# MaurizioFD/RecSys2019_DeepLearning_Evaluation

Measured on NVIDIA H100. Metric: ItemKNN cosine top-K rows/sec, higher is better.
Workload: dtype i32 counts + f32

## Files before the change

### recsys2019_deeplearning_evaluation_b200/csrc/sim_k1d.cuh

```cuda

constexpr int D_THREADS = 512;
constexpr int D_WARPS = D_THREADS / 32;
constexpr int D_ROWS = 4;
constexpr int D_TILE_LOG2 = 10;

constexpr int K1D_GAPS = 6;
__device__ __forceinline__ int k1d_gap(const int4& c, int e) {
  const int w = e < 2 ? c.y : (e < 4 ? c.z : c.w);
  return (e & 1) ? (int)((unsigned)w >> 16) : (w & 0xffff);
}

struct K1DShared {
  int item, nbuf, cnt, nibsum, tstop, chunk_end, chunk_cnt;
  int ncand, expect;
  CtaSelectSmem<256> sel;
};

__device__ __forceinline__ unsigned nib_ge3(unsigned w) { return (((w | (w >> 1)) >> 2) | (w & (w >> 1))) & 0x11111111u; }
__device__ __forceinline__ unsigned nib_eq2(unsigned w) { return (w >> 1) & ~w & ~(w >> 2) & ~(w >> 3) & 0x11111111u; }
__device__ __forceinline__ unsigned nib_eq1(unsigned w) { return w & ~(w >> 1) & ~(w >> 2) & ~(w >> 3) & 0x11111111u; }
__device__ __forceinline__ unsigned nib_level(unsigned w, int level) {
  return level >= 3 ? nib_ge3(w) : (level == 2 ? nib_eq2(w) : nib_eq1(w));
}
__device__ __forceinline__ int nib_sum(unsigned w) {
  const unsigned b = (w & 0x0F0F0F0Fu) + ((w >> 4) & 0x0F0F0F0Fu);
  return (int)__dp4a(b, 0x01010101u, 0u);
}

__device__ u64 d_select(u64* buf, int n, int K, K1DShared* ds, int* n_out) {
  const int tid = threadIdx.x;
  __syncthreads();
  if (n <= K) { *n_out = n; return 0ull; }
  const auto sel_key = [&](int q, u64& key) {
    key = buf[q];
    return true;
  };
  const u64 thr = radix_select<u64, 8, true>(CtaSelect<D_THREADS, 256>(ds->sel), n, K, sel_key).thr;
  u64 keep[8];
#pragma unroll
  for (int q = 0; q < 8; ++q) {
    const int i = q * D_THREADS + tid;
    const u64 k = i < n ? buf[i] : 0ull;
    keep[q] = k >= thr ? k : 0ull;
  }
  if (tid == 0) ds->cnt = 0;
  __syncthreads();
#pragma unroll
  for (int q = 0; q < 8; ++q)
    if (keep[q]) buf[atomicAdd(&ds->cnt, 1)] = keep[q];
  __syncthreads();
  *n_out = ds->cnt;
  return thr;
}

template <int F>
__global__ void __launch_bounds__(D_THREADS, 2) sim_k1d_kernel(const KParams p) {
  extern __shared__ __align__(16) unsigned char smem_raw[];
  __shared__ K1DShared ds;
  const int tid = threadIdx.x, lane = tid & 31, warp = tid >> 5;
  const int W = p.bm_words;
  const int Wr = (p.n_cols + 7) >> 3;
  const int ntile = p.ntile;
  unsigned* acc = reinterpret_cast<unsigned*>(smem_raw);
  u64* buf = reinterpret_cast<u64*>(smem_raw + (size_t)W * 4);
  float* tbs = reinterpret_cast<float*>(buf + p.cap_d);
  int* tcnt = reinterpret_cast<int*>(tbs + ntile + 1);

  for (int i = tid; i < W; i += D_THREADS) acc[i] = 0u;
  for (int i = tid; i <= ntile; i += D_THREADS) tbs[i] = p.tbnd[i];
  for (int i = tid; i < ntile; i += D_THREADS) tcnt[i] = 0;
  long long prof_t = p.prof ? clock64() : 0;
  const int K = p.K;
  const int n_items = p.n_range_dev ? *p.n_range_dev : p.n_range;

  for (;;) {
    __syncthreads();
    if (tid == 0) { ds.item = atomicAdd(p.counter, 1); ds.nbuf = 0; ds.nibsum = 0; ds.ncand = 0; }
    __syncthreads();
    const int item = ds.item;
    if (item >= n_items) break;
    const int4 wi = __ldg(p.worklist + item);
    const int col = wi.x, lc = wi.y, cs = wi.z, ce = wi.w;
    const size_t out_base = (size_t)lc * K;
    const float Ai = p.A[col];
    const int adds = __ldg(p.col_adds + col);

    for (int k0 = cs + warp * 32; k0 < ce; k0 += D_WARPS * 32) {
      const int nrows = min(32, ce - k0);
      int2 seg = make_int2(0, 0);
      if (lane < nrows) seg = __ldg(p.csc_seg + k0 + lane);
      const int hl = lane & 15, hh = lane >> 4;
      for (int r0 = 0; r0 < nrows; r0 += 2 * D_ROWS) {
        int4 v[D_ROWS];
        int rs[D_ROWS], rn[D_ROWS];
#pragma unroll
        for (int q = 0; q < D_ROWS; ++q) {
          const int r = r0 + 2 * q + hh;
          rs[q] = __shfl_sync(0xffffffffu, seg.x, r & 31);
          rn[q] = __shfl_sync(0xffffffffu, seg.y, r & 31);
          if (r >= nrows) rn[q] = 0;
          if (hl < rn[q]) v[q] = __ldg(p.csr_idx1 + (size_t)rs[q] + hl);
        }
#pragma unroll
        for (int q = 0; q < D_ROWS; ++q) {
          int c0 = 0;
          for (;;) {
            if (c0 + hl < rn[q]) {
              int j = v[q].x;
              if (j < p.n_cols && j != col) atomicAdd(&acc[j >> 3], 1u << ((j & 7) << 2));
#pragma unroll
              for (int e = 0; e < K1D_GAPS; ++e) {
                const int g = k1d_gap(v[q], e);
                j += g;
                if (g && j < p.n_cols && j != col) atomicAdd(&acc[j >> 3], 1u << ((j & 7) << 2));
              }
            }
            c0 += 16;
            if (c0 >= rn[q]) break;
            if (c0 + hl < rn[q]) v[q] = __ldg(p.csr_idx1 + (size_t)rs[q] + c0 + hl);
          }
        }
      }
    }
    __syncthreads();
    PROF_MARK(1);

    {
      int ns = 0;
      unsigned* cand = reinterpret_cast<unsigned*>(buf);
      const int cand_cap = p.cap_d;
      const uint4* acc4 = reinterpret_cast<const uint4*>(acc);
      for (int i4 = tid; i4 < ((Wr + 3) >> 2); i4 += D_THREADS) {
        const uint4 w4 = acc4[i4];
        if (!(w4.x | w4.y | w4.z | w4.w)) continue;
        const unsigned ww[4] = {w4.x, w4.y, w4.z, w4.w};
        unsigned bytes = 0u, any = 0u, m[4];
#pragma unroll
        for (int e = 0; e < 4; ++e) {
          bytes += (ww[e] & 0x0F0F0F0Fu) + ((ww[e] >> 4) & 0x0F0F0F0Fu);
          m[e] = nib_ge3(ww[e]);
          any |= m[e];
        }
        ns += (int)__dp4a(bytes, 0x01010101u, 0u);
        if (any) {
          const int c3 = __popc(m[0]) + __popc(m[1]) + __popc(m[2]) + __popc(m[3]);
          atomicAdd(&tcnt[(i4 * 4) >> (D_TILE_LOG2 - 3)], c3);
          int pos = atomicAdd(&ds.ncand, c3);
          if (pos + c3 <= cand_cap) {
#pragma unroll
            for (int e = 0; e < 4; ++e) {
              unsigned mm = m[e];
              while (mm) {
                const int q = (__ffs(mm) - 1) >> 2;
                mm &= mm - 1;
                cand[pos++] = ((unsigned)((i4 * 4 + e) * 8 + q) << 4) | ((ww[e] >> (q << 2)) & 15u);
              }
            }
          }
        }
      }
      ns = __reduce_add_sync(0xffffffffu, ns);
      if (lane == 0 && ns) atomicAdd(&ds.nibsum, ns);
    }
    __syncthreads();
    const bool forced = p.fail_every > 0 && (lc % p.fail_every) == 0;
    if (ds.nibsum != adds || forced) {
      __syncthreads();
      if (tid == 0) p.redo[atomicAdd(p.fail, 1)] = lc;
      for (int i = tid; i < (W >> 2); i += D_THREADS) reinterpret_cast<int4*>(acc)[i] = make_int4(0, 0, 0, 0);
      for (int i = tid; i < ntile; i += D_THREADS) tcnt[i] = 0;
      continue;
    }
    PROF_MARK(2);

    u64 thr = 0ull;
    int n_have = 0;
    const int n3 = ds.ncand;
    const bool collected = n3 <= p.cap_d;
    if (collected) {
      const unsigned* cand = reinterpret_cast<const unsigned*>(buf);
      u64 keys[4];
#pragma unroll
      for (int q = 0; q < 4; ++q) {
        const int t = q * D_THREADS + tid;
        keys[q] = 0ull;
        if (t < n3) {
          const unsigned cd = cand[t];
          const int2 bn = __ldg(p.BN + (cd >> 4));
          const float sv = sim_value<F>(p, (float)(cd & 15u), Ai, __int_as_float(bn.x));
          if (sv > 0.f) keys[q] = (((u64)__float_as_uint(sv)) << 32) | (u64)(0xFFFFFFFFu - (unsigned)bn.y);
        }
      }
      __syncthreads();
#pragma unroll
      for (int q = 0; q < 4; ++q)
        if (keys[q]) buf[atomicAdd(&ds.nbuf, 1)] = keys[q];
      for (int i = tid; i < ntile; i += D_THREADS) tcnt[i] = 0;
      __syncthreads();
      n_have = ds.nbuf;
      if (n_have >= K) {
        const float fl = sim_value<F>(p, 3.f, Ai, tbs[ntile]) * (1.f - 1e-6f);
        if (fl > 0.f) thr = ((u64)__float_as_uint(fl)) << 32;
      }
      PROF_MARK(3);
    }
#pragma unroll 1
    for (int level = collected ? 2 : 3; level >= 1; --level) {
      int t_end = ntile;
      if (level < 3) {
        if (thr == 0ull) {
          t_end = ntile;
        } else {
          const float tsim = __uint_as_float((unsigned)(thr >> 32));
          if (tid == 0) ds.tstop = ntile;
          __syncthreads();
          for (int t = tid; t < ntile; t += D_THREADS)
            if (!(sim_value<F>(p, (float)level, Ai, tbs[t]) >= tsim)) atomicMin(&ds.tstop, t);
          __syncthreads();
          t_end = ds.tstop;
          __syncthreads();
        }
        if (t_end == 0) continue;
        const int w_end = min(Wr, t_end << (D_TILE_LOG2 - 3));
        for (int i = tid; i < w_end; i += D_THREADS) {
          const unsigned w = acc[i];
          if (!w) continue;
          const int c = __popc(nib_level(w, level));
          if (c) atomicAdd(&tcnt[i >> (D_TILE_LOG2 - 3)], c);
        }
        __syncthreads();
      }
      int t0 = 0;
      while (t0 < t_end) {
        if (tid == 0) {
          int t1 = t0, c = 0;
          while (t1 < t_end && n_have + c + tcnt[t1] <= p.cap_d) { c += tcnt[t1]; ++t1; }
          ds.chunk_end = t1;
          ds.chunk_cnt = c;
        }
        __syncthreads();
        const int t1 = ds.chunk_end;
        if (t1 == t0) {
          int kept;
          const u64 t2 = d_select(buf, n_have, K, &ds, &kept);
          thr = max(thr, t2);
          if (tid == 0) ds.nbuf = kept;
          n_have = kept;
          __syncthreads();
          continue;
        }
        if (ds.chunk_cnt > 0) {
          const int w_lo = t0 << (D_TILE_LOG2 - 3), w_hi = min(Wr, t1 << (D_TILE_LOG2 - 3));
          for (int i = w_lo + tid; i < w_hi; i += D_THREADS) {
            const unsigned w = acc[i];
            if (!w) continue;
            unsigned m = nib_level(w, level);
            while (m) {
              const int q = (__ffs(m) - 1) >> 2;
              m &= m - 1;
              const int j = i * 8 + q;
              const float d = (float)((w >> (q << 2)) & 15u);
              const int2 bn = __ldg(p.BN + j);
              const float sv = sim_value<F>(p, d, Ai, __int_as_float(bn.x));
              const u64 key = (((u64)__float_as_uint(sv)) << 32) | (u64)(0xFFFFFFFFu - (unsigned)bn.y);
              if (sv > 0.f && key >= thr) buf[atomicAdd(&ds.nbuf, 1)] = key;
            }
          }
        }
        __syncthreads();
        n_have = ds.nbuf;
        t0 = t1;
      }
      for (int i = tid; i < ntile; i += D_THREADS) tcnt[i] = 0;
      __syncthreads();
      if (n_have >= K) {
        if (level == 3 && thr == 0ull) {
          const float fl = sim_value<F>(p, 3.f, Ai, tbs[ntile]) * (1.f - 1e-6f);
          if (fl > 0.f) thr = ((u64)__float_as_uint(fl)) << 32;
        } else if (level == 2 && n_have > K) {
          int kept;
          const u64 t2 = d_select(buf, n_have, K, &ds, &kept);
          thr = max(thr, t2);
          if (tid == 0) ds.nbuf = kept;
          n_have = kept;
          __syncthreads();
        }
      }
      if (level == 3) PROF_MARK(3); else if (level == 2) PROF_MARK(4); else PROF_MARK(5);
    }

    {
      int kept;
      d_select(buf, n_have, K, &ds, &kept);
      n_have = kept;
    }
    for (int t = tid; t < n_have; t += D_THREADS) {
      const u64 k64 = buf[t];
      emit_entry(p, out_base + t, (int)(0xFFFFFFFFu - (unsigned)k64), __uint_as_float((unsigned)(k64 >> 32)));
    }
    for (int t = n_have + tid; t < K; t += D_THREADS) {
      emit_entry(p, out_base + t, -1, 0.f);
    }
    if (tid == 0) emit_count(p, lc, n_have);
    for (int i = tid; i < (W >> 2); i += D_THREADS) reinterpret_cast<int4*>(acc)[i] = make_int4(0, 0, 0, 0);
    PROF_MARK(6);
  }
}


#ifndef B200_U_THREADS
#define B200_U_THREADS 256
#endif
#ifndef B200_U_CTAS
#define B200_U_CTAS 4
#endif
#ifndef B200_U_STEPS
#define B200_U_STEPS 4
#endif
#ifndef B200_U_STAGE
#define B200_U_STAGE 1024
#endif
constexpr int U_THREADS = B200_U_THREADS;
constexpr int U_WARPS = U_THREADS / 32;
constexpr int U_CTAS = B200_U_CTAS;
constexpr int U_STEPS = B200_U_STEPS;
constexpr int U_STAGE = B200_U_STAGE;

__host__ __device__ __forceinline__ int k1d_window_size(int n, int c) { return ((n - 1) >> 1) + ((n & 1) == 0 && c < (n >> 1) ? 1 : 0); }
__host__ __device__ __forceinline__ int k1d_upper_words(int n) { return (((n >> 1) + 7) / 8 + 3) / 4 * 4; }
constexpr int OWN_SPILLED = (int)0x80000000u;

struct K1DUpShared {
  int item, nibsum, ncand, nst;
  unsigned long long base;
};

__global__ void __launch_bounds__(U_THREADS, U_CTAS) sim_k1d_upper_kernel(const KParams p) {
  extern __shared__ __align__(16) unsigned char smem_raw[];
  __shared__ K1DUpShared us;
  const int tid = threadIdx.x, lane = tid & 31, warp = tid >> 5;
  const int n = p.n_cols;
  const int W = k1d_upper_words(n);
  unsigned* acc = reinterpret_cast<unsigned*>(smem_raw);
  unsigned* stage = acc + W;
  for (int i = tid; i < W; i += U_THREADS) acc[i] = 0u;
  if (blockIdx.x == 0 && tid == 0 && p.fail_every > 0) atomicExch(p.pair_fail, 1);
  long long prof_t = p.prof ? clock64() : 0;

  for (;;) {
    __syncthreads();
    if (tid == 0) {
      us.item = *(volatile int*)p.pair_fail ? p.n_range : atomicAdd(p.counter, 1);
      us.nibsum = 0; us.ncand = 0; us.nst = 0;
    }
    __syncthreads();
    const int item = us.item;
    if (item >= p.n_range) break;
    const int4 wi = __ldg(p.worklist_up + item);
    const int col = wi.x, adds = wi.y, cs = wi.z, ce = wi.w;
    const int size_c = k1d_window_size(n, col);

    for (int k0 = cs + warp * 32; k0 < ce; k0 += U_WARPS * 32) {
      const int nrows = min(32, ce - k0);
      int2 seg = make_int2(0, 0);
      if (lane < nrows) seg = __ldg(p.csc_win + k0 + lane);
      const unsigned nz = __ballot_sync(0xffffffffu, seg.y > 0);
      const int nr = __popc(nz);
      const int src = lane < nr ? (int)__fns(nz, 0, lane + 1) : 0;
      const int rstart = __shfl_sync(0xffffffffu, seg.x, src);
      const int sy = __shfl_sync(0xffffffffu, seg.y, src);
      const int rn = lane < nr ? sy : 0;
      int end = rn;
#pragma unroll
      for (int off = 1; off < 32; off <<= 1) {
        const int t = __shfl_up_sync(0xffffffffu, end, off);
        if (lane >= off) end += t;
      }
      const int beg = end - rn;
      const int total = __shfl_sync(0xffffffffu, end, 31);
      for (int b0 = 0; b0 < total; b0 += 32 * U_STEPS) {
        int4 v[U_STEPS];
#pragma unroll
        for (int q = 0; q < U_STEPS; ++q) {
          const int base = b0 + 32 * q, f = base + lane;
          const unsigned before = __ballot_sync(0xffffffffu, lane < nr && end <= base);
          const unsigned ends = __reduce_or_sync(0xffffffffu, (lane < nr && end > base && end - base < 32) ? (1u << (end - base)) : 0u);
          const int row = (__popc(before) + __popc(ends & ((2u << lane) - 1u))) & 31;
          const int rb = __shfl_sync(0xffffffffu, beg, row), rs = __shfl_sync(0xffffffffu, rstart, row);
          if (f < total) v[q] = __ldg(p.csr_idx1 + (size_t)rs + (f - rb));
        }
#pragma unroll
        for (int q = 0; q < U_STEPS; ++q) {
          if (b0 + 32 * q + lane < total) {
            unsigned t = (unsigned)(v[q].x - col - 1);
            if (t < (unsigned)size_c) atomicAdd(&acc[t >> 3], 1u << ((t & 7) << 2));
#pragma unroll
            for (int e = 0; e < K1D_GAPS; ++e) {
              const unsigned g = (unsigned)k1d_gap(v[q], e);
              t += g;
              if (g && t < (unsigned)size_c) atomicAdd(&acc[t >> 3], 1u << ((t & 7) << 2));
            }
          }
        }
      }
    }
    __syncthreads();
    PROF_MARK(8);

    {
      int ns = 0;
      uint4* acc4 = reinterpret_cast<uint4*>(acc);
      for (int i4 = tid; i4 < ((((size_c + 7) >> 3) + 3) >> 2); i4 += U_THREADS) {
        const uint4 w4 = acc4[i4];
        if (!(w4.x | w4.y | w4.z | w4.w)) continue;
        acc4[i4] = make_uint4(0u, 0u, 0u, 0u);
        const unsigned ww[4] = {w4.x, w4.y, w4.z, w4.w};
        unsigned bytes = 0u, any = 0u, m[4];
#pragma unroll
        for (int e = 0; e < 4; ++e) {
          bytes += (ww[e] & 0x0F0F0F0Fu) + ((ww[e] >> 4) & 0x0F0F0F0Fu);
          m[e] = nib_ge3(ww[e]);
          any |= m[e];
        }
        ns += (int)__dp4a(bytes, 0x01010101u, 0u);
        if (any) {
          const int c3 = __popc(m[0]) + __popc(m[1]) + __popc(m[2]) + __popc(m[3]);
          int pos = atomicAdd(&us.ncand, c3);
          const bool staged = pos + c3 <= U_STAGE;
          unsigned long long g = 0ull;
          if (staged) atomicAdd(&us.nst, c3);
          else g = atomicAdd(p.n_loose, (unsigned long long)c3);
#pragma unroll
          for (int e = 0; e < 4; ++e) {
            unsigned mm = m[e];
            while (mm) {
              const int q = (__ffs(mm) - 1) >> 2;
              mm &= mm - 1;
              int j = col + 1 + (i4 * 4 + e) * 8 + q;
              if (j >= n) j -= n;
              const unsigned cd = ((unsigned)j << 4) | ((ww[e] >> (q << 2)) & 15u);
              if (staged) {
                stage[pos++] = cd;
              } else {
                atomicAdd(p.deg + j, 1);
                if (g < (unsigned long long)p.loose_cap) p.loose[g] = ((u64)col << 32) | cd;
                else atomicExch(p.pair_fail, 1);
                ++g;
              }
            }
          }
        }
      }
      ns = __reduce_add_sync(0xffffffffu, ns);
      if (lane == 0 && ns) atomicAdd(&us.nibsum, ns);
    }
    __syncthreads();
    const int nst = us.nst;
    if (tid == 0) {
      if (us.nibsum != adds) atomicExch(p.pair_fail, 1);
      us.base = nst ? atomicAdd(p.n_own, (unsigned long long)nst) : 0ull;
      if (us.base + nst > (unsigned long long)p.pair_cap) atomicExch(p.pair_fail, 1);
      p.own_off[col] = (int)us.base;
      p.own_n[col] = nst | (us.ncand > nst ? OWN_SPILLED : 0);
    }
    __syncthreads();
    const unsigned long long base = us.base;
    if (base + nst <= (unsigned long long)p.pair_cap)
      for (int t = tid; t < nst; t += U_THREADS) {
        const unsigned cd = stage[t];
        p.own[base + t] = cd;
        atomicAdd(p.deg + (cd >> 4), 1);
      }
    PROF_MARK(9);
  }
}

__global__ void k1d_pair_scatter_kernel(const KParams p) {
  const long long t0 = blockIdx.x * (long long)blockDim.x + threadIdx.x, nt = (long long)gridDim.x * blockDim.x;
  if (*p.pair_fail) {
    for (long long q = t0; q <= p.n_cols; q += nt) p.deg[q] = 0;
    return;
  }
  const int i = (int)(t0 >> 5), lane = threadIdx.x & 31;
  if (i < p.n_cols) {
    const int s = p.own_off[i], n = p.own_n[i] & ~OWN_SPILLED;
    for (int t = lane; t < n; t += 32) {
      const unsigned cd = p.own[s + t], j = cd >> 4;
      p.mir[p.mir_off[j] + atomicSub(p.deg + j, 1) - 1] = ((unsigned)i << 4) | (cd & 15u);
    }
  }
  const long long nl = (long long)min(*p.n_loose, (u64)p.loose_cap);
  for (long long q = t0; q < nl; q += nt) {
    const u64 e = p.loose[q];
    const unsigned cd = (unsigned)e, j = cd >> 4;
    p.mir[p.mir_off[j] + atomicSub(p.deg + j, 1) - 1] = ((unsigned)(e >> 32) << 4) | (cd & 15u);
  }
}

constexpr int S_WARPS = 4;
constexpr int S_CTAS = 6;
constexpr int S_CAP = 4 * D_THREADS;
constexpr int S_ILP = 12;
__host__ __device__ __forceinline__ int k1d_select_warp_bytes(int sel_cap) { return 256 * 4 + (sel_cap * 8 + 15) / 16 * 16; }

template <int F>
__global__ void __launch_bounds__(32 * S_WARPS, S_CTAS) sim_k1d_select_kernel(const KParams p) {
  extern __shared__ __align__(16) unsigned char smem_raw[];
  unsigned char* mine = smem_raw + (size_t)(threadIdx.x >> 5) * k1d_select_warp_bytes(p.sel_cap);
  int* hist = reinterpret_cast<int*>(mine);
  u64* keys = reinterpret_cast<u64*>(mine + 256 * 4);
  const int lane = threadIdx.x & 31;
  const int item = blockIdx.x * S_WARPS + (threadIdx.x >> 5);
  if (item >= p.n_range) return;
  const int4 wi = __ldg(p.worklist + item);
  if (*(volatile int*)p.pair_fail) {
    if (lane == 0) { p.wl_redo[item] = wi; atomicAdd(p.n_redo, 1); }
    return;
  }
  long long prof_t = p.prof ? clock64() : 0;
  const int col = wi.x, lc = wi.y, K = p.K;
  const int so = p.own_off[col], no = p.own_n[col];
  const int sm = p.mir_off[col], n = no + (p.mir_off[col + 1] - sm);
  bool ok = no >= 0 && n <= p.sel_cap;
  int n_have = 0;
  if (ok) {
    const float Ai = p.A[col];
    const unsigned* own = p.own + so;
    const unsigned* mir = p.mir + sm - no;
    for (int t0 = 0; t0 < n; t0 += 32 * S_ILP) {
      unsigned cd[S_ILP];
      int2 bn[S_ILP];
#pragma unroll
      for (int q = 0; q < S_ILP; ++q) {
        const int t = t0 + 32 * q + lane;
        cd[q] = t < n ? (t < no ? own : mir)[t] : 0u;
      }
#pragma unroll
      for (int q = 0; q < S_ILP; ++q)
        if (t0 + 32 * q + lane < n) bn[q] = __ldg(p.BN + (cd[q] >> 4));
#pragma unroll
      for (int q = 0; q < S_ILP; ++q) {
        u64 key = 0ull;
        if (t0 + 32 * q + lane < n) {
          const float sv = sim_value<F>(p, (float)(cd[q] & 15u), Ai, __int_as_float(bn[q].x));
          if (sv > 0.f) key = (((u64)__float_as_uint(sv)) << 32) | (u64)(0xFFFFFFFFu - (unsigned)bn[q].y);
        }
        const unsigned b = __ballot_sync(0xffffffffu, key != 0ull);
        if (key) keys[n_have + __popc(b & ((1u << lane) - 1u))] = key;
        n_have += __popc(b);
      }
    }
    ok = false;
    if (n_have >= K) {
      const float fl = sim_value<F>(p, 3.f, Ai, p.tbnd[p.ntile]) * (1.f - 1e-6f);
      if (fl > 0.f) ok = !(sim_value<F>(p, 2.f, Ai, p.lvl_b2) >= fl) && !(sim_value<F>(p, 1.f, Ai, p.lvl_b1) >= fl);
    }
  }
  PROF_MARK_WARP(10);
  if (!ok) {
    if (lane == 0) p.wl_redo[atomicAdd(p.n_redo, 1)] = wi;
    return;
  }
  __syncwarp();
  const auto sel_key = [&](int q, u64& key) {
    key = keys[q];
    return true;
  };
  const u64 thr = n_have > K ? radix_select<u64, 8, true>(WarpSelect{hist}, n_have, K, sel_key).thr : 0ull;
  const size_t out_base = (size_t)lc * K;
  int kept = 0;
  for (int t0 = 0; t0 < n_have; t0 += 32) {
    const int t = t0 + lane;
    const u64 k64 = t < n_have ? keys[t] : 0ull;
    const bool keep = t < n_have && k64 >= thr;
    const unsigned b = __ballot_sync(0xffffffffu, keep);
    if (keep)
      emit_entry(p, out_base + kept + __popc(b & ((1u << lane) - 1u)), (int)(0xFFFFFFFFu - (unsigned)k64),
                 __uint_as_float((unsigned)(k64 >> 32)));
    kept += __popc(b);
  }
  for (int t = kept + lane; t < K; t += 32) emit_entry(p, out_base + t, -1, 0.f);
  if (lane == 0) emit_count(p, lc, kept);
  PROF_MARK_WARP(11);
}

__global__ void k1d_tile_bounds_kernel(const int2* __restrict__ BN, int n_cols, int ntile, float* tb) {
  const int t = blockIdx.x * blockDim.x + threadIdx.x;
  if (t > ntile) return;
  tb[t] = __int_as_float(BN[min(t << D_TILE_LOG2, n_cols - 1)].x);
}

__device__ __forceinline__ int k1d_row_entry(const int* __restrict__ row, int len, int n_cols, int m) {
  return m < len ? row[m] : row[m - len] + n_cols;
}

template <class Emit>
__device__ __forceinline__ int k1d_row_chunks(const int* __restrict__ row, int len, int copies, int n_cols, Emit emit) {
  const int total = copies * len;
  int nch = 0;
  for (int m = 0; m < total; ++nch) {
    const int base = k1d_row_entry(row, len, n_cols, m++);
    unsigned long long g14 = 0ull;
    unsigned g56 = 0u;
    for (int e = 0, prev = base; e < K1D_GAPS && m < total; ++e, ++m) {
      const int j = k1d_row_entry(row, len, n_cols, m);
      if (j - prev >= 65536) break;
      if (e < 4) g14 |= (unsigned long long)(j - prev) << (16 * e); else g56 |= (unsigned)(j - prev) << (16 * (e - 4));
      prev = j;
    }
    emit(nch, make_int4(base, (int)(unsigned)g14, (int)(unsigned)(g14 >> 32), (int)g56));
  }
  return nch;
}

__global__ void k1d_row_len_kernel(const int* __restrict__ csr_ptr, const int* __restrict__ csr_idx, int n_rows, int copies, int n_cols,
                                   int* nchunk) {
  const int u = blockIdx.x * blockDim.x + threadIdx.x;
  if (u >= n_rows) return;
  nchunk[u] = k1d_row_chunks(csr_idx + csr_ptr[u], csr_ptr[u + 1] - csr_ptr[u], copies, n_cols, [](int, int4) {});
}

__global__ void k1d_row_fill_kernel(const int* __restrict__ csr_ptr, const int* __restrict__ csr_idx, const int* __restrict__ poff,
                                    int n_rows, int copies, int n_cols, int4* rows) {
  const int u = (int)((blockIdx.x * (long long)blockDim.x + threadIdx.x) >> 3), l = threadIdx.x & 7;
  if (u >= n_rows) return;
  int4* out = rows + poff[u];
  k1d_row_chunks(csr_idx + csr_ptr[u], csr_ptr[u + 1] - csr_ptr[u], copies, n_cols, [=](int ch, int4 c) { if ((ch & 7) == l) out[ch] = c; });
}

__device__ __forceinline__ int k1d_chunk_of(const int4* __restrict__ row, int nch, int m, int v) {
  int lo = m / (K1D_GAPS + 1), hi = nch;
  if (lo + 1 == nch || row[lo + 1].x > v) return lo;
  while (hi - lo > 1) {
    const int mid = (lo + hi) >> 1;
    if (row[mid].x <= v) lo = mid; else hi = mid;
  }
  return lo;
}

__global__ void k1d_csc_rows_kernel(const int* __restrict__ csc_ptr, const int* __restrict__ csc_idx, const int* __restrict__ csr_ptr,
                                    const int* __restrict__ csr_idx, const int* __restrict__ csc_pos, const int* __restrict__ poff,
                                    const int4* __restrict__ rows, int n_cols, int2* seg, int* col_adds, int2* win,
                                    unsigned long long* win_work, int* iota) {
  const int c = (blockIdx.x * blockDim.x + threadIdx.x) >> 5, lane = threadIdx.x & 31;
  if (c >= n_cols) return;
  const int bound = c + k1d_window_size(n_cols, c);
  unsigned long long w = 0;
  int full = 0;
  for (int q = csc_ptr[c] + lane; q < csc_ptr[c + 1]; q += 32) {
    const int u = csc_idx[q];
    const int r0 = csr_ptr[u], len = csr_ptr[u + 1] - r0, s = poff[u], nch = poff[u + 1] - s;
    const int* row = csr_idx + r0;
    seg[q] = make_int2(s, k1d_chunk_of(rows + s, nch, len - 1, row[len - 1]) + 1);
    full += len - 1;
    if (!win) continue;
    const int k = csc_pos[q] - r0;
    int lo = k + 1, hi = k + len;
    while (lo < hi) {
      const int mid = (lo + hi) >> 1;
      if (k1d_row_entry(row, len, n_cols, mid) <= bound) lo = mid + 1; else hi = mid;
    }
    int2 d = make_int2(0, 0);
    if (lo > k + 1) {
      const int first = k1d_chunk_of(rows + s, nch, k + 1, k1d_row_entry(row, len, n_cols, k + 1));
      d = make_int2(s + first, k1d_chunk_of(rows + s, nch, lo - 1, k1d_row_entry(row, len, n_cols, lo - 1)) - first + 1);
    }
    win[q] = d;
    w += (unsigned long long)(lo - k - 1);
  }
  full = __reduce_add_sync(0xffffffffu, full);
  if (lane == 0) col_adds[c] = full;
  if (!win) return;
#pragma unroll
  for (int off = 16; off > 0; off >>= 1) w += __shfl_xor_sync(0xffffffffu, w, off);
  if (lane == 0) { win_work[c] = w; iota[c] = c; }
}

__global__ void k1d_upper_worklist_kernel(const int* __restrict__ perm, const unsigned long long* __restrict__ work,
                                          const int* __restrict__ csc_ptr, int n_cols, int4* wl) {
  const int k = blockIdx.x * blockDim.x + threadIdx.x;
  if (k >= n_cols) return;
  const int c = perm[k];
  wl[k] = make_int4(c, (int)(unsigned)work[k], csc_ptr[c], csc_ptr[c + 1]);
}
```

Before: 14.41 million.

## Software-pipeline CSR loads and prefetch next work item in upper k1d kernel

The upper co-occurrence kernel now double-buffers its CSR index loads, so the next batch is issued while the current one is counted, and it prefetches the next row-segment descriptor. It also claims and loads the next work item during the current one, which removes a barrier-guarded fetch at the top of each iteration. Counting becomes branchless `red.shared.add`: invalid entries add zero to a dummy word. U_STEPS drops from 4 to 3 to limit register pressure from the double buffer. The cost is extra shared-memory atomic traffic from the dummy adds and more complex control flow.

```diff
diff --git a/recsys2019_deeplearning_evaluation_b200/csrc/sim_k1d.cuh b/recsys2019_deeplearning_evaluation_b200/csrc/sim_k1d.cuh
--- a/recsys2019_deeplearning_evaluation_b200/csrc/sim_k1d.cuh
+++ b/recsys2019_deeplearning_evaluation_b200/csrc/sim_k1d.cuh
@@ -315,7 +315,7 @@
 #define B200_U_CTAS 4
 #endif
 #ifndef B200_U_STEPS
-#define B200_U_STEPS 4
+#define B200_U_STEPS 3
 #endif
 #ifndef B200_U_STAGE
 #define B200_U_STAGE 1024
@@ -332,8 +332,15 @@
 
 struct K1DUpShared {
   int item, nibsum, ncand, nst;
+  int4 wi;
   unsigned long long base;
 };
+
+static_assert(U_STAGE >= 32, "an entry that does not count adds 0 to shared word `lane`");
+__device__ __forceinline__ void k1d_up_count(unsigned acc_s, int lane, unsigned t, bool ok) {
+  const unsigned word = ok ? t >> 3 : (unsigned)lane, inc = ok ? __funnelshift_l(0u, 1u, t << 2) : 0u;
+  asm volatile("red.shared.add.u32 [%0], %1;" :: "r"(acc_s + (word << 2)), "r"(inc) : "memory");
+}
 
 __global__ void __launch_bounds__(U_THREADS, U_CTAS) sim_k1d_upper_kernel(const KParams p) {
   extern __shared__ __align__(16) unsigned char smem_raw[];
@@ -343,43 +350,64 @@
   const int W = k1d_upper_words(n);
   unsigned* acc = reinterpret_cast<unsigned*>(smem_raw);
   unsigned* stage = acc + W;
+  const unsigned acc_s = (unsigned)__cvta_generic_to_shared(acc);
   for (int i = tid; i < W; i += U_THREADS) acc[i] = 0u;
   if (blockIdx.x == 0 && tid == 0 && p.fail_every > 0) atomicExch(p.pair_fail, 1);
   long long prof_t = p.prof ? clock64() : 0;
+  if (tid == 0) {
+    const int it = atomicAdd(p.counter, 1);
+    us.item = *(volatile int*)p.pair_fail ? p.n_range : it;
+    if (us.item < p.n_range) us.wi = __ldg(p.worklist_up + us.item);
+    us.nibsum = 0; us.ncand = 0; us.nst = 0;
+  }
+  __syncthreads();
 
   for (;;) {
-    __syncthreads();
-    if (tid == 0) {
-      us.item = *(volatile int*)p.pair_fail ? p.n_range : atomicAdd(p.counter, 1);
-      us.nibsum = 0; us.ncand = 0; us.nst = 0;
-    }
-    __syncthreads();
     const int item = us.item;
     if (item >= p.n_range) break;
-    const int4 wi = __ldg(p.worklist_up + item);
+    const int4 wi = us.wi;
     const int col = wi.x, adds = wi.y, cs = wi.z, ce = wi.w;
     const int size_c = k1d_window_size(n, col);
-
-    for (int k0 = cs + warp * 32; k0 < ce; k0 += U_WARPS * 32) {
-      const int nrows = min(32, ce - k0);
-      int2 seg = make_int2(0, 0);
-      if (lane < nrows) seg = __ldg(p.csc_win + k0 + lane);
-      const unsigned nz = __ballot_sync(0xffffffffu, seg.y > 0);
-      const int nr = __popc(nz);
-      const int src = lane < nr ? (int)__fns(nz, 0, lane + 1) : 0;
-      const int rstart = __shfl_sync(0xffffffffu, seg.x, src);
-      const int sy = __shfl_sync(0xffffffffu, seg.y, src);
-      const int rn = lane < nr ? sy : 0;
-      int end = rn;
-#pragma unroll
-      for (int off = 1; off < 32; off <<= 1) {
-        const int t = __shfl_up_sync(0xffffffffu, end, off);
-        if (lane >= off) end += t;
-      }
-      const int beg = end - rn;
-      const int total = __shfl_sync(0xffffffffu, end, 31);
-      for (int b0 = 0; b0 < total; b0 += 32 * U_STEPS) {
-        int4 v[U_STEPS];
+    int it_next = 0, failed = 0;
+    if (tid == 0) {
+      it_next = atomicAdd(p.counter, 1);
+      failed = *(volatile int*)p.pair_fail;
+    }
+
+    {
+      const unsigned sz = (unsigned)size_c;
+      int k0 = cs + warp * 32;
+      const auto desc = [&](int k) {
+        int2 s = make_int2(0, 0);
+        if (k + lane < ce) s = __ldg(p.csc_win + k + lane);
+        return s;
+      };
+      int rstart = 0, beg = 0, end = 0, nr = 0, total = 0, b0 = 0;
+      const auto open = [&](int2 seg) {
+        const unsigned nz = __ballot_sync(0xffffffffu, seg.y > 0);
+        nr = __popc(nz);
+        const int src = lane < nr ? (int)__fns(nz, 0, lane + 1) : 0;
+        rstart = __shfl_sync(0xffffffffu, seg.x, src);
+        const int sy = __shfl_sync(0xffffffffu, seg.y, src);
+        const int rn = lane < nr ? sy : 0;
+        end = rn;
+#pragma unroll
+        for (int off = 1; off < 32; off <<= 1) {
+          const int t = __shfl_up_sync(0xffffffffu, end, off);
+          if (lane >= off) end += t;
+        }
+        beg = end - rn;
+        total = __shfl_sync(0xffffffffu, end, 31);
+        b0 = 0;
+      };
+      bool live = k0 < ce;
+      int2 seg_next = make_int2(0, 0);
+      if (live) {
+        const int2 seg = desc(k0);
+        seg_next = desc(k0 + U_WARPS * 32);
+        open(seg);
+      }
+      const auto issue = [&](int4 (&v)[U_STEPS]) {
 #pragma unroll
         for (int q = 0; q < U_STEPS; ++q) {
           const int base = b0 + 32 * q, f = base + lane;
@@ -387,22 +415,49 @@
           const unsigned ends = __reduce_or_sync(0xffffffffu, (lane < nr && end > base && end - base < 32) ? (1u << (end - base)) : 0u);
           const int row = (__popc(before) + __popc(ends & ((2u << lane) - 1u))) & 31;
           const int rb = __shfl_sync(0xffffffffu, beg, row), rs = __shfl_sync(0xffffffffu, rstart, row);
-          if (f < total) v[q] = __ldg(p.csr_idx1 + (size_t)rs + (f - rb));
-        }
+          v[q] = f < total ? __ldg(p.csr_idx1 + (size_t)rs + (f - rb)) : make_int4(col, 0, 0, 0);
+        }
+        b0 += 32 * U_STEPS;
+        if (b0 >= total) {
+          k0 += U_WARPS * 32;
+          live = k0 < ce;
+          if (live) {
+            const int2 seg = seg_next;
+            seg_next = desc(k0 + U_WARPS * 32);
+            open(seg);
+          }
+        }
+      };
+      const auto count = [&](const int4 (&v)[U_STEPS]) {
 #pragma unroll
         for (int q = 0; q < U_STEPS; ++q) {
-          if (b0 + 32 * q + lane < total) {
-            unsigned t = (unsigned)(v[q].x - col - 1);
-            if (t < (unsigned)size_c) atomicAdd(&acc[t >> 3], 1u << ((t & 7) << 2));
-#pragma unroll
-            for (int e = 0; e < K1D_GAPS; ++e) {
-              const unsigned g = (unsigned)k1d_gap(v[q], e);
-              t += g;
-              if (g && t < (unsigned)size_c) atomicAdd(&acc[t >> 3], 1u << ((t & 7) << 2));
-            }
+          unsigned t = (unsigned)(v[q].x - col - 1);
+          k1d_up_count(acc_s, lane, t, t < sz);
+#pragma unroll
+          for (int e = 0; e < K1D_GAPS; ++e) {
+            const unsigned g = (unsigned)k1d_gap(v[q], e);
+            t += g;
+            k1d_up_count(acc_s, lane, t, g != 0u && t < sz);
           }
         }
-      }
+      };
+      int4 va[U_STEPS], vb[U_STEPS];
+      bool have_a = live;
+      if (live) issue(va);
+      while (have_a) {
+        const bool have_b = live;
+        if (live) issue(vb);
+        count(va);
+        if (!have_b) break;
+        have_a = live;
+        if (live) issue(va);
+        count(vb);
+      }
+    }
+    int4 wi_next = make_int4(0, 0, 0, 0);
+    if (tid == 0) {
+      it_next = failed ? p.n_range : it_next;
+      if (it_next < p.n_range) wi_next = __ldg(p.worklist_up + it_next);
     }
     __syncthreads();
     PROF_MARK(8);
@@ -454,6 +509,7 @@
       ns = __reduce_add_sync(0xffffffffu, ns);
       if (lane == 0 && ns) atomicAdd(&us.nibsum, ns);
     }
+    if (tid == 0) { us.item = it_next; us.wi = wi_next; }
     __syncthreads();
     const int nst = us.nst;
     if (tid == 0) {
@@ -471,6 +527,7 @@
         p.own[base + t] = cd;
         atomicAdd(p.deg + (cd >> 4), 1);
       }
+    if (tid == 0) { us.nibsum = 0; us.ncand = 0; us.nst = 0; }
     PROF_MARK(9);
   }
 }
```

Measured after the change: 16.24 million (median of 6 runs). 1.13x the previous value.
